# BaamPark/DistributedDataParallel-Cifar10

Measured on AMD Instinct MI355X. Metric: images/sec (whole node) CIFAR-10 ResNet at 1/2/4/8 MI355X; scaling efficiency, higher is better.
Workload: dtype bf16; 1 GPU; model=NetResDeep(n_chans1=32, n_blocks=10), global_batch=32, per_rank_batch=32, image=3x32x32, parallelism=dp1, optimizer=SGD(lr=1e-2)

## Files before the change

### distributeddataparallel_cifar10_amd/csrc/engine.hip

```cpp
#include <rccl/rccl.h>

#include <cstdio>
#include <cstdlib>
#include <cstring>
#include <map>
#include <string>
#include <vector>

#include "netresdeep_kernels.hip"
#include "xgmi_allreduce.hip"
#include "netresdeep_pks.hip"

namespace {

thread_local std::string g_err;

#define HIPCK(x)                                                                   \
  do {                                                                             \
    hipError_t e_ = (x);                                                           \
    if (e_ != hipSuccess) {                                                        \
      g_err = std::string(#x) + ": " + hipGetErrorString(e_);                      \
      return -1;                                                                   \
    }                                                                              \
  } while (0)
// ... 222 lines not shown
  else
    hipLaunchKernelGGL(xg::k_xgmi_ar_sgd<false>, dim3(xg::AR_NB), dim3(xg::AR_T), 0, e->st, cx, e->peers,
                       (const float*)cx.grads, (float*)nullptr, e->qa.err + 1, 1, e->ar_deadline);
  HIPCK(hipGetLastError());
  return 0;
}

static int pks_grid(int B) { return (B + 7) / 8 * 8 * pks::S; }
static int pks_live(int B) { return B * pks::S; }

static int coresident_budget(int per_cu, int ncu, int n_share, bool full_device) {
  const int slots = per_cu * ncu;
  const int margin = per_cu > 1 ? ncu : (full_device && n_share <= 1 ? 0 : 1);
  return (slots - margin) / std::max(n_share, 1);
}
static int share_budget(const Engine* e) {
  return e->shared_device > 1 ? coresident_budget(e->per_cu, e->ncu, e->shared_device, false) : e->resident;
}
static int seg_ch(const Engine* e) { return e->shared_device > 1 ? 256 : 128; }

static bool fc_in_step_for(const Engine* e, int B) {
  return e->fc_in_step && pks_live(B) + pks::N_FCW <= share_budget(e);
}
static int reduce_grid(const Engine* e, int nred_plus) {
  return e->shared_device > 1 ? std::min(nred_plus, share_budget(e)) : nred_plus;
}

static bool prologue_ok(const Engine* e, int B) {
  if (!e->persistent || !e->prologue) return false;
  if (e->comm_on && e->in.comm_mode != 2) return false;
  if (!fc_in_step_for(e, B)) return false;
  return pks_live(B) + std::max(pks::N_FCW, pks::prologue_segments(seg_ch(e))) <= share_budget(e);
}

static int enqueue_pks_step(Engine* e, int B, int s, bool prev) {
  Ctx cx = e->base;
  cx.B = B;
  const bool multi = e->comm_on, xgmi = multi && e->in.comm_mode == 2;
  if (xgmi && !e->peers_open) {
    g_err = "xGMI all-reduce: peers not mapped (call dca_engine_ipc_open first)";
    return -1;
  }
  if (pks_live(B) > share_budget(e)) {
    g_err = "persistent engine: " + std::to_string(pks_live(B)) + " step workgroups (batch " + std::to_string(B) +
            ") exceed the co-residency budget of " + std::to_string(share_budget(e)) + " per rank";
    return -1;
  }
  pks::RedAr ra{};
  ra.peers = e->peers;
  ra.err = e->qa.err + 1;
  ra.deadline = e->ar_deadline;
  ra.mode = !multi ? 0 : (xgmi ? 2 : 1);
  const bool fc = fc_in_step_for(e, B);
  ra.fc_in_step = pks::ra_flags(fc, prev, s, 0);
  ra.seg_ch = seg_ch(e);
  const int extra = fc ? std::max(pks::N_FCW, prev ? pks::prologue_segments(ra.seg_ch) : 0) : 0;
  const dim3 grid(pks_grid(B) + extra);
  const dim3 blk(pks::NTH);
  if (e->bf && prev)
    hipLaunchKernelGGL((pks::k_pks_step<0, true>), grid, blk, pks::Plan<0>::TOTAL, e->st, cx, e->qa, ra);
  else if (e->bf)
    hipLaunchKernelGGL((pks::k_pks_step<0, false>), grid, blk, pks::Plan<0>::TOTAL, e->st, cx, e->qa, ra);
  else if (prev)
    hipLaunchKernelGGL((pks::k_pks_step<1, true>), grid, blk, pks::Plan<1>::TOTAL, e->st, cx, e->qa, ra);
  else
    hipLaunchKernelGGL((pks::k_pks_step<1, false>), grid, blk, pks::Plan<1>::TOTAL, e->st, cx, e->qa, ra);
  HIPCK(hipGetLastError());
  return 0;
}

static int enqueue_pks_reduce(Engine* e, int B, int chunk, int part) {
  Ctx cx = e->base;
  cx.B = B;
  const bool multi = e->comm_on, xgmi = multi && e->in.comm_mode == 2;
  if (part != 2) {
    pks::RedAr ra{};
    ra.peers = e->peers;
    ra.err = e->qa.err + 1;
    ra.deadline = e->ar_deadline;
    ra.mode = !multi ? 0 : (xgmi ? 2 : 1);
    const bool fc = fc_in_step_for(e, B);
    ra.fc_in_step = pks::ra_flags(fc, false, 0, chunk);
    ra.seg_ch = seg_ch(e);
    const dim3 rgrid(reduce_grid(e, pks::reduce_segments(fc, ra.seg_ch) + 1));
    const int lean = !fc ? 0 : (ra.mode == 0 ? 1 : (ra.mode == 2 ? 2 : 0));
    const size_t lds = pks::stage_floats(B) * 4;
    if (lean == 1)
      hipLaunchKernelGGL(pks::k_pks_reduce_ar<1>, rgrid, dim3(256), lds, e->st, cx, e->qa, B * pks::S, ra);
    else if (lean == 2)
      hipLaunchKernelGGL(pks::k_pks_reduce_ar<2>, rgrid, dim3(256), lds, e->st, cx, e->qa, B * pks::S, ra);
    else
      hipLaunchKernelGGL(pks::k_pks_reduce_ar<0>, rgrid, dim3(256), lds, e->st, cx, e->qa, B * pks::S, ra);
  }
  if (multi && !xgmi) {
    if (part == 0) NCCK(ncclAllReduce(cx.grads, cx.grads, FLAT_N, ncclFloat32, ncclSum, e->comm, e->st));
    if (part != 1) hipLaunchKernelGGL(e->kapply, dim3(64), dim3(NT), 0, e->st, cx, 1);
  }
  HIPCK(hipGetLastError());
  return 0;
}

static int enqueue_step_persistent(Engine* e, int B, int part) {
  if (part != 2 && enqueue_pks_step(e, B, 0, false)) return -1;
  return enqueue_pks_reduce(e, B, 1, part);
}

static int enqueue_step(Engine* e, int B, int part = 0);
static int enqueue_chunk(Engine* e, int B, int chunk) {
  if (!prologue_ok(e, B)) {
    for (int s = 0; s < chunk; ++s)
      if (enqueue_step(e, B)) return -1;
    return 0;
  }
  for (int s = 0; s < chunk; ++s)
    if (enqueue_pks_step(e, B, s, s > 0)) return -1;
  return enqueue_pks_reduce(e, B, chunk, 0);
}

static int enqueue_step(Engine* e, int B, int part) {
  if (e->persistent) return enqueue_step_persistent(e, B, part);
  Ctx cx = e->base;
  cx.B = B;
  if (part == 2) {
    hipLaunchKernelGGL(e->kapply, dim3(64), dim3(NT), 0, e->st, cx, 1);
    HIPCK(hipGetLastError());
    return 0;
  }
  const int nparts = B * e->TPI, nw = B * (16 / e->RW);
  const int nslab = 9 * nw + nparts;
  const dim3 blk(NT);
  hipLaunchKernelGGL(e->kstem, dim3(nparts), blk, e->s_stem, e->st, cx);
  for (int i = 1; i < NBLK; ++i) hipLaunchKernelGGL(e->kfwd, dim3(nparts), blk, e->s_fwd, e->st, cx, i);
  hipLaunchKernelGGL(e->khead1, dim3(nparts), blk, e->s_head1, e->st, cx);
  hipLaunchKernelGGL(e->khead2, dim3(nparts), blk, e->s_head2, e->st, cx);
  for (int i = NBLK - 1; i >= 0; --i) {
    const int extra = (i == NBLK - 1) ? N_FC_WG : nw;
    size_t lds = (i == 0) ? e->s_dgrad0 : e->s_dgrad;
    lds = std::max(lds, (i < NBLK - 1) ? e->s_wgrad : e->s_fc);
    hipLaunchKernelGGL(e->kbwd, dim3(nparts + extra), blk, lds, e->st, cx, i);
    if (i == NBLK - 1 && e->comm_on && part == 0 && e->in.comm_mode == 0) {
      HIPCK(hipEventRecord(e->evA, e->st));
      HIPCK(hipStreamWaitEvent(e->cst, e->evA, 0));
      NCCK(ncclAllReduce(cx.grads, cx.grads, BUCKET_A_END, ncclFloat32, ncclSum, e->comm, e->cst));
    }
  }
  const int nother = cx.fuse_sgd ? 64 : 0;
  hipLaunchKernelGGL(e->kred, dim3(N_TRUNK_RED_WG + N_STEM_RED_WG + nother + 1), blk, 0, e->st, cx, nslab, nparts);
  if (e->comm_on && part == 0 && e->in.comm_mode == 2) return enqueue_xgmi_sgd(e, cx);
  if (e->comm_on && part == 0) {
    HIPCK(hipEventRecord(e->evB, e->st));
    HIPCK(hipStreamWaitEvent(e->cst, e->evB, 0));
    NCCK(ncclAllReduce(cx.grads + OFF_CONVW, cx.grads + OFF_CONVW, FLAT_N - OFF_CONVW, ncclFloat32, ncclSum, e->comm,
                       e->cst));
    HIPCK(hipEventRecord(e->evC, e->cst));
    HIPCK(hipStreamWaitEvent(e->st, e->evC, 0));
    hipLaunchKernelGGL(e->kapply, dim3(64), blk, 0, e->st, cx, 1);
  }
  HIPCK(hipGetLastError());
  return 0;
}

}


using dca::Engine;

extern "C" {

// ... 636 lines not shown
```

### distributeddataparallel_cifar10_amd/csrc/netresdeep_pks.hip

```cpp

namespace dca {
#ifndef DCA_DETAIL_FWD
#define DCA_DETAIL_FWD 5
#endif
#ifndef DCA_DETAIL_BWD
#define DCA_DETAIL_BWD 5
#endif
namespace pks {

constexpr int S = 4;
constexpr int RS = 16 / S;
constexpr int NW = 2 * RS;
constexpr int NTH = 64 * NW;
constexpr int GSTR = 64 + 2 * 512;
constexpr int LMAX = 64 * S;
constexpr int NNT = (18 + NW - 1) / NW;
constexpr int RND_HEAD = 10;
constexpr unsigned SPIN_LIMIT = 1u << 17;
constexpr int RB = 64;
constexpr int cmax(int a, int b) { return a > b ? a : b; }

struct Args {
  unsigned long long* gran;
  unsigned* bnx;
// ... 251 lines not shown
      if (ok) need &= ~(1u << k);
    }
#pragma unroll
    for (int p = 0; p < 2; ++p)
      if (xh[p][1] == htag && xh[p][3] == htag) need &= ~(1u << (8 + p));
    if (__all(need == 0)) break;
    if (spins >= SPIN_LIMIT) {
      if (lane == 0) atomicOr(pa.err, 1u << (round & 31));
      break;
    }
  }
#pragma unroll
  for (int e = 0; e < 4; ++e) sv[e] = 0.f;
#pragma unroll
  for (int k = 0; k < KS; ++k) {
    const bool valid = 4 * wv + sub + 4 * NW * k < G;
#pragma unroll
    for (int e = 0; e < 4; ++e) sv[e] += valid ? __uint_as_float(xa[k][e]) : 0.f;
  }
#pragma unroll
  for (int p = 0; p < 2; ++p) {
    hv[2 * p] = __uint_as_float(xh[p][0]);
    hv[2 * p + 1] = __uint_as_float(xh[p][2]);
  }
}
__device__ __forceinline__ void xchg_wait(const Args& pa, int round, int epoch, int G, float* cred, bool halo,
                                          int Lsrc, int which, int h, float (&hv)[4]) {
  const int t = threadIdx.x, lane = t & 63;
  const int wv = __builtin_amdgcn_readfirstlane(t >> 6);
  const unsigned tag = tagof(epoch, round);
  float sv[4];
  const unsigned btag = bn_tag(epoch, round);
  if (G <= 4 * NW) sweep_wait<1>(pa, round, wv, lane, G, btag, sv, halo, Lsrc, which, h, tag, hv);
  else if (G <= 8 * NW) sweep_wait<2>(pa, round, wv, lane, G, btag, sv, halo, Lsrc, which, h, tag, hv);
  else if (G <= 16 * NW) sweep_wait<4>(pa, round, wv, lane, G, btag, sv, halo, Lsrc, which, h, tag, hv);
  else sweep_wait<8>(pa, round, wv, lane, G, btag, sv, halo, Lsrc, which, h, tag, hv);
#pragma unroll
  for (int e = 0; e < 4; ++e) {
    sv[e] = xsum_rows(sv[e]);
  }
  if (lane < 16) {
#pragma unroll
    for (int e = 0; e < 4; ++e) cred[(4 * lane + e) * NW + wv] = sv[e];
  }
}
__device__ __forceinline__ float slot_total(const float* cred, int slot) {
  static_assert(NW == 8 && RS == 4, "slot-major combine layout: 8 waves, 4 rows");
  const f32x4 u = *(const f32x4*)(cred + slot * NW), w = *(const f32x4*)(cred + slot * NW + 4);
  float a = u[0];
  a += u[1];
  a += u[2];
  a += u[3];
  a += w[0];
  a += w[1];
  a += w[2];
  a += w[3];
  return a;
}

__device__ __forceinline__ void st4_wt(void* p, f32x4 v) {
  asm volatile("global_store_dwordx4 %0, %1, off sc1\n\ts_nop 1" ::"v"(p), "v"(v) : "memory");
}
__device__ __forceinline__ void st2_wt(float* p, float a, float b) {
  typedef float f2_ __attribute__((ext_vector_type(2)));
  asm volatile("global_store_dwordx2 %0, %1, off sc1" ::"v"(p), "v"(f2_{a, b}) : "memory");
}
__device__ __forceinline__ void st1_wt(float* p, float v) {
  __hip_atomic_store((unsigned*)p, __float_as_uint(v), __ATOMIC_RELAXED, __HIP_MEMORY_SCOPE_AGENT);
}
__device__ __forceinline__ void st4r_wt(float* rowp, int h, int lane, const float (&v)[4]) {
  st4_wt(rowp + h * 256 + lane * 4, f32x4{v[0], v[1], v[2], v[3]});
}
__device__ __forceinline__ void st4r(float* rowp, int h, int lane, const float (&v)[4]) {
  *(f32x4*)(rowp + h * 256 + lane * 4) = f32x4{v[0], v[1], v[2], v[3]};
}
__device__ __forceinline__ void ld4r(const float* rowp, int h, int lane, float (&v)[4]) {
  const f32x4 u = *(const f32x4*)(rowp + h * 256 + lane * 4);
  v[0] = u[0];
  v[1] = u[1];
  v[2] = u[2];
  v[3] = u[3];
}

template <int P>
__device__ __forceinline__ void wgrad_acc(const unsigned short* dyT, const unsigned short* xT, f32x4 (&wacc)[NNT][2],
                                          int wv, int lane) {
  using PL = Plan<P>;
  const int c = lane & 15, q = lane >> 4;
  constexpr int DYO = PL::DYT_PL / 2, XTO = PL::XT_PL / 2;
#pragma unroll
  for (int s = 0; s < RS / 2; ++s) {
    const int row = 2 * s + (q >> 1), c0 = 8 * (q & 1);
    const int ao0 = c * PL::DYT_S + row * 16 + c0, ao1 = (16 + c) * PL::DYT_S + row * 16 + c0;
    const bf16x8 a0 = *(const bf16x8*)(dyT + ao0);
    const bf16x8 a1 = *(const bf16x8*)(dyT + ao1);
    bf16x8 a0l = a0, a1l = a1;
    if constexpr (P == 1) {
      a0l = *(const bf16x8*)(dyT + DYO + ao0);
      a1l = *(const bf16x8*)(dyT + DYO + ao1);
    }
#pragma unroll
    for (int j = 0; j < NNT; ++j) {
      const int nt = wv + NW * j;
      if (nt < 18) {
        const int tap = nt >> 1, cih = nt & 1, kh = tap / 3, kw = tap % 3;
        const int bo = (kw * 32 + 16 * cih + c) * PL::XT_S + (row + kh) * 16 + c0;
        const bf16x8 b = *(const bf16x8*)(xT + bo);
        bf16x8 bl = b;
        if constexpr (P == 1) bl = *(const bf16x8*)(xT + XTO + bo);
        wacc[j][0] = mma3<P>(a0, a0l, b, bl, wacc[j][0]);
        wacc[j][1] = mma3<P>(a1, a1l, b, bl, wacc[j][1]);
      }
    }
  }
}
__device__ __forceinline__ void xt_put(unsigned short* xT, int XT_S, int xrow, int ch, int q, unsigned b0, unsigned b1,
                                       unsigned b2, unsigned b3) {
  const int rowoff = xrow * 16 + 4 * q;
  unsigned short* p1 = xT + (32 + ch) * XT_S + rowoff;
  *(uint2*)p1 = uint2{b0 | (b1 << 16), b2 | (b3 << 16)};
  unsigned short* p0 = xT + ch * XT_S + rowoff;
  p0[1] = (unsigned short)b0;
  *(unsigned*)(p0 + 2) = b1 | (b2 << 16);
  if (q < 3) p0[4] = (unsigned short)b3;
  unsigned short* p2 = xT + (64 + ch) * XT_S + rowoff;
  if (q > 0) p2[-1] = (unsigned short)b0;
  *(unsigned*)p2 = b1 | (b2 << 16);
  p2[2] = (unsigned short)b3;
}
template <int P>
__device__ __forceinline__ void xt_row(unsigned short* xT, int xrow, int q, int ch, const float (&x)[4]) {
  using PL = Plan<P>;
  unsigned hb[4], lb[4];
#pragma unroll
  for (int i = 0; i < 4; ++i) {
    const unsigned short hi = bfbits(x[i]);
    hb[i] = hi;
    lb[i] = P == 1 ? bf_lo(x[i], hi) : 0u;
  }
  xt_put(xT, PL::XT_S, xrow, ch, q, hb[0], hb[1], hb[2], hb[3]);
  if constexpr (P == 1) xt_put(xT + PL::XT_PL / 2, PL::XT_S, xrow, ch, q, lb[0], lb[1], lb[2], lb[3]);
}
template <int P>
__device__ __forceinline__ void xr_row(char* XR, int xrow, int q, int ch, const float (&v)[4]) {
  using PL = Plan<P>;
#pragma unroll
  for (int i = 0; i < 4; ++i) st1r<P>(XR, PL::XR_PL, xrow * 18 + 4 * q + i + 1, ch, v[i]);
}

template <int P>
__device__ __forceinline__ void wt_dma(char* wt, const unsigned short* src, int wv, int lane) {
  constexpr int BYTES = (P + 1) * PKW_PLANE * 2, NCH = (BYTES + 1023) / 1024;
  static_assert(BYTES == (P + 1) * Plan<P>::WT_PL, "record layout of pkw matches the LDS weight planes");
#pragma unroll
  for (int m = 0; m < (NCH + NW - 1) / NW; ++m) {
    const int ck = wv + NW * m;
    if (ck < NCH && ck * 1024 + lane * 16 < BYTES)
      __builtin_amdgcn_global_load_lds((const __attribute__((address_space(1))) void*)((const char*)src + ck * 1024 + lane * 16),
                                       (__attribute__((address_space(3))) void*)(wt + ck * 1024), 16, 0, 0);
  }
}
template <int P>
__device__ __forceinline__ void wt_copy_sc1(char* wt, const unsigned short* src) {
  constexpr int BYTES = (P + 1) * PKW_PLANE * 2, N16 = BYTES / 16, R = (N16 + NTH - 1) / NTH;
  const __amdgpu_buffer_rsrc_t rs = __builtin_amdgcn_make_buffer_rsrc((void*)src, (short)0, BYTES, 0x00020000);
  v4u v[R];
// ... 97 lines not shown
__host__ __device__ __forceinline__ int ra_chunk(const RedAr& ra) { return (ra.fc_in_step >> 16) & 255; }
__host__ __device__ __forceinline__ int ra_flags(int fc, int prev, int s, int chunk) {
  return (fc ? 1 : 0) | (prev ? 2 : 0) | (s << 8) | (chunk << 16);
}
__device__ __forceinline__ int step_epoch(const Args& pa, const RedAr& ra) {
  return (int)(((unsigned)*pa.epoch + (unsigned)ra_s(ra)) % EPOCH_WRAP);
}
__device__ __forceinline__ char* rbase(const RedAr& ra, int q) { return ra.peers.base[q] + xg::REGION_BYTES; }
__device__ __forceinline__ float* rslab(const RedAr& ra, int q, int par) {
  return (float*)(rbase(ra, q) + xg::FLAG_BYTES) + (size_t)par * xg::SLAB_FLOATS;
}

template <int NTH>
__device__ bool seg_exchange(const Ctx& cx, const RedAr& ra, int b, float* segv, int len, int off, int ep0, int* s_ep) {
  const int t = threadIdx.x, W = cx.ws, me = cx.rank;
  int* myflags = (int*)rbase(ra, me);
  const unsigned long long t_in = __builtin_amdgcn_s_memrealtime();
  if (t == 0) {
    s_ep[0] = xg::next_ep(ep0);
    s_ep[1] = xg::failed(ra.err);
  }
  __syncthreads();
  const int ep = s_ep[0], par = ep & 1;
  if (s_ep[1]) return false;
  constexpr int SYS = 17;
  const __amdgpu_buffer_rsrc_t mine =
      __builtin_amdgcn_make_buffer_rsrc(rslab(ra, me, par), (short)0, (int)(xg::SLAB_FLOATS * 4), 0x00020000);
  for (int k = 4 * t; k < len; k += 4 * NTH)
    __builtin_amdgcn_raw_buffer_store_b128(__builtin_bit_cast(xg::v4u, *(const f32x4*)(segv + k)), mine,
                                           4 * (off + k), 0, SYS);
  asm volatile("s_waitcnt vmcnt(0)" ::: "memory");
  __syncthreads();
  if (t < W) xg::flag_store((int*)rbase(ra, t) + me * NSEG_MAX + b, ep);
  if (t < W) xg::wait_flag(myflags + t * NSEG_MAX + b, ep, ra.deadline, ra.err);
  __syncthreads();
  if (t == 0) s_ep[1] = xg::failed(ra.err);
  __syncthreads();
  if (s_ep[1]) return false;
  if (t == 0 && b < seg_layout(ra.seg_ch).r_ts && ra.peers.ticks != nullptr) {
    atomicAdd(ra.peers.ticks, __builtin_amdgcn_s_memrealtime() - t_in);
    atomicAdd(ra.peers.ticks + 1, 1ull);
  }
  for (int k = 4 * t; k < len; k += 4 * NTH) {
    *(f32x4*)(segv + k) = rank_sum(W, [&](int q) {
      const __amdgpu_buffer_rsrc_t rs = __builtin_amdgcn_make_buffer_rsrc(rslab(ra, q, par), (short)0,
                                                                          (int)(xg::SLAB_FLOATS * 4), 0x00020000);
      return __builtin_bit_cast(f32x4, __builtin_amdgcn_raw_buffer_load_b128(rs, 4 * (off + k), 0, SYS));
    });
  }
  __syncthreads();
  return true;
}

__device__ __forceinline__ int seg_pidx(const SegLayout& G, int b, int k) {
  if (b < G.r_ts) {
    const bool stem = b >= G.r_trunk;
    const int e = (stem ? b - G.r_trunk : b) * G.ch + k, ii = k & 3;
    if (e >= (stem ? SSLAB_N : WSLAB_N)) return -1;
    const int tt = e >> 8, ln = (e >> 2) & 63, mt = tt & 1, nt = tt >> 1;
    if (!stem) return OFF_CONVW + (16 * mt + 4 * (ln >> 4) + ii) * 288 + (16 * (nt & 1) + (ln & 15)) * 9 + (nt >> 1);
    if (e < 1024) {
      const int kk = 16 * nt + (ln & 15);
      return kk < 27 ? OFF_C1W + (16 * mt + 4 * (ln >> 4) + ii) * 27 + kk : -1;
    }
    return e < 1056 ? OFF_C1B + (e - 1024) : -1;
  }
  if (b < G.fct) {
    const int fb = b - G.r_ts;
    return OFF_FC1W + (16 * (fb & 1) + (k >> 6)) * 2048 + 64 * (fb >> 1) + (k & 63);
  }
  if (b == G.fct) {
    if (k < 32) return OFF_FC1B + k;
    if (k < 352) return OFF_FC2W + ((k - 32) >> 5) * 32 + ((k - 32) & 31);
    return k < 362 ? OFF_FC2B + (k - 352) : -1;
  }
  return k < 64 ? (k < 32 ? OFF_BNW : OFF_BNB) + (k & 31) : -2 - (k - 64);
}

__device__ __forceinline__ f32x4 ld4_sc1(const float* base, int bytes, int off_floats) {
  const __amdgpu_buffer_rsrc_t rs = __builtin_amdgcn_make_buffer_rsrc((void*)base, (short)0, bytes, 0x00020000);
  return __builtin_bit_cast(f32x4, __builtin_amdgcn_raw_buffer_load_b128(rs, 4 * off_floats, 0, 16));
}

template <int NTH, int CH>
__device__ __forceinline__ void seg_chunk(const Ctx& cx, const Args& pa, const SegLayout& Ls, int b, int nslab,
                                          float* segv, f32x4* red) {
  constexpr int NS = CH / 4, VG = 2048 / CH, NG = NTH / NS, VPG = VG / NG, NU = 128 / VG, HG = VG / 2;
  static_assert(NG * VPG == VG && (VPG == 1 || VPG == 2), "512- or 256-thread reducers");
  const int t = threadIdx.x;
  const bool stem = b >= Ls.r_trunk;
  const int chunk = stem ? b - Ls.r_trunk : b;
  const int slot = t % NS, grp = t / NS, e0 = chunk * CH + slot * 4;
  const float* src = stem ? cx.SSLAB : pa.tslab;
  const int stride = stem ? SSLAB_N : WSLAB_N;
  const int ec = e0 < stride ? e0 : stride - 4;
  f32x4 sacc[VPG];
#pragma unroll
  for (int vp = 0; vp < VPG; ++vp) sacc[vp] = z4();
  for (int k0 = 0; k0 < nslab; k0 += 128) {
#pragma unroll
    for (int vp = 0; vp < VPG; ++vp) {
      const int gv = grp + NG * vp;
      f32x4 v[NU];
#pragma unroll
      for (int u = 0; u < NU; ++u) {
        const int k = k0 + gv + VG * u;
        const int kc = k < nslab ? k : nslab - 1;
        v[u] = ld4(src + (size_t)kc * stride + ec);
      }
#pragma unroll
      for (int u = 0; u < NU; ++u)
        if (k0 + gv + VG * u < nslab) sacc[vp] += v[u];
    }
  }
  red[t] = VPG == 2 ? sacc[0] + sacc[VPG - 1] : sacc[0];
  __syncthreads();
  if (t < NS) {
    f32x4 tot;
    if constexpr (VPG == 2) {
      tot = red[t];
#pragma unroll
      for (int g = 1; g < HG; ++g) tot += red[NS * g + t];
    } else {
      tot = red[t] + red[NS * HG + t];
#pragma unroll
      for (int g = 1; g < HG; ++g) tot += red[NS * g + t] + red[NS * (g + HG) + t];
    }
    *(f32x4*)(segv + slot * 4) = e0 < stride ? tot : z4();
  }
}

template <int NTH>
__device__ __forceinline__ void pkw_trunk_chunks_wt(const Ctx& cx, const float* wnew, int e_base, int len) {
  for (int t = threadIdx.x; t < 64 * (len / 128); t += NTH) {
    const int hf = t >> 6, j = t & 63, kind = j >> 4, idx = j & 15;
    const int e0 = e_base + hf * 128, tt = e0 >> 8, h = (e0 >> 7) & 1, mt = tt & 1, nt = tt >> 1;
    const int tap = nt >> 1, cih = nt & 1;
    const float* w = wnew + hf * 128;
    unsigned short v[8];
    int dst;
    if (kind < 2) {
      const int col = idx >> 1, qq = idx & 1, co = 16 * mt + 8 * h + col;
#pragma unroll
      for (int j8 = 0; j8 < 8; ++j8) {
        const float x = w[64 * (col >> 2) + 4 * (8 * qq + j8) + (col & 3)];
        const unsigned short hi = bfbits(x);
        v[j8] = kind == 0 ? hi : bf_lo(x, hi);
      }
      dst = (kind == 1 ? PKW_PLANE : 0) + pkw_elem(tap * 32 + co, 16 * cih + 8 * qq);
    } else {
      const int cl = idx;
#pragma unroll
      for (int c8 = 0; c8 < 8; ++c8) {
        const float x = w[64 * (c8 >> 2) + 4 * cl + (c8 & 3)];
        const unsigned short hi = bfbits(x);
        v[c8] = kind == 2 ? hi : bf_lo(x, hi);
      }
      dst = PKW_DGRAD + (kind == 3 ? PKW_PLANE : 0) + pkw_elem((8 - tap) * 32 + 16 * cih + cl, 16 * mt + 8 * h);
    }
    st4_wt(cx.pkw + dst, __builtin_bit_cast(f32x4, v4u{v[0] | ((unsigned)v[1] << 16), v[2] | ((unsigned)v[3] << 16),
                                                       v[4] | ((unsigned)v[5] << 16), v[6] | ((unsigned)v[7] << 16)}));
  }
}

template <int NTH, bool WT = false, int LEAN = 0>
__device__ void seg_process(const Ctx& cx, const Args& pa, const RedAr& ra, int b, int nslab, float* segv,
                            f32x4* red, float* stage, int* s_ep, int sslot, int swg) {
  const int t = threadIdx.x, B = cx.B;
  const int mode = LEAN == 1 ? 0 : (LEAN == 2 ? 2 : ra.mode);
  const SegLayout Ls = seg_layout(ra.seg_ch);
  const int len = seg_len(Ls, b), off = seg_off(Ls, b);
  const int ep0 = mode >= 2 && t == 0 ? xg::flag_load((const int*)rbase(ra, cx.rank) + cx.rank * NSEG_MAX + b) : 0;
  constexpr int KMAX = SEG_MAX / NTH;
  int pid[KMAX];
  float pold[KMAX];
#pragma unroll
  for (int i = 0; i < KMAX; ++i) {
    const int k = t + NTH * i;
    pid[i] = k < len && mode != 3 ? seg_pidx(Ls, b, k) : -1;
    pold[i] = cx.params[pid[i] >= 0 ? pid[i] : 0];
  }
  if (mode == 3) {
    for (int k = t; k < len; k += NTH) segv[k] = off + k < ra.st_n ? ra.st_src[off + k] : 0.f;
  } else if (b < Ls.r_ts) {
    if (Ls.ch == 128) seg_chunk<NTH, 128>(cx, pa, Ls, b, nslab, segv, red);
    else seg_chunk<NTH, 256>(cx, pa, Ls, b, nslab, segv, red);
  } else if (!LEAN && b < Ls.fct) {
    const int fb = b - Ls.r_ts, f = fb >> 1, j0 = 16 * (fb & 1);
    float* dh_s = stage;
    float* p_s = stage + B * 32;
    constexpr int MD = (64 * 8 + NTH - 1) / NTH, MP = (64 * 16 + NTH - 1) / NTH;
    f32x4 dh4[MD], p4[MP];
#pragma unroll
    for (int m = 0; m < MD; ++m) {
      const int idx = t + NTH * m;
      dh4[m] = ld4_sc1(cx.HDH, 64 * 32 * 4, 4 * (idx < B * 8 ? idx : 0));
    }
#pragma unroll
    for (int m = 0; m < MP; ++m) {
      const int idx = t + NTH * m, ic = idx < B * 16 ? idx : 0, bb = ic >> 4, k4 = ic & 15;
      p4[m] = ld4_sc1(cx.HP, 64 * 2048 * 4, bb * 2048 + 64 * f + 4 * k4);
    }
#pragma unroll
    for (int m = 0; m < MD; ++m)
      if (t + NTH * m < B * 8) st4(dh_s + 4 * (t + NTH * m), dh4[m]);
#pragma unroll
    for (int m = 0; m < MP; ++m)
      if (t + NTH * m < B * 16) st4(p_s + 4 * (t + NTH * m), p4[m]);
    __syncthreads();
    if (t < 256) {
      const int jl = t >> 4, kk = 4 * (t & 15);
      f32x4 a0 = z4();
#pragma unroll 8
      for (int bb = 0; bb < B; ++bb) a0 += dh_s[bb * 32 + j0 + jl] * ld4(p_s + bb * 64 + kk);
      st4(segv + jl * 64 + kk, a0);
    }
  } else if (!LEAN && b == Ls.fct) {
    float* hh_s = stage;
    float* dl_s = stage + B * 32;
    float* dh_s = dl_s + B * 16;
    for (int idx = t; idx < B * 8; idx += NTH) {
      st4(hh_s + 4 * idx, ld4_sc1(cx.HH, 64 * 32 * 4, 4 * idx));
      st4(dh_s + 4 * idx, ld4_sc1(cx.HDH, 64 * 32 * 4, 4 * idx));
    }
    for (int idx = t; idx < B * 10; idx += NTH) {
      const __amdgpu_buffer_rsrc_t rs = __builtin_amdgcn_make_buffer_rsrc((void*)cx.HDL, (short)0, 64 * 16 * 4, 0x00020000);
      dl_s[(idx / 10) * 16 + idx % 10] = __builtin_bit_cast(float, __builtin_amdgcn_raw_buffer_load_b32(rs, 4 * idx, 0, 16));
    }
    __syncthreads();
    for (int idx = t; idx < FCT_LEN; idx += NTH) {
      float sv = 0.f;
      if (idx < 32) {
#pragma unroll 8
        for (int bb = 0; bb < B; ++bb) sv += dh_s[bb * 32 + idx];
      } else if (idx < 352) {
        const int o = (idx - 32) >> 5, jj = (idx - 32) & 31;
#pragma unroll 8
        for (int bb = 0; bb < B; ++bb) sv += dl_s[bb * 16 + o] * hh_s[bb * 32 + jj];
      } else if (idx < 362) {
        const int o = idx - 352;
#pragma unroll 8
        for (int bb = 0; bb < B; ++bb) sv += dl_s[bb * 16 + o];
      }
      segv[idx] = sv;
    }
  } else {
    for (int idx = t; idx < BNT_LEN; idx += NTH) {
      float sv;
      if (idx < 64) {
        sv = pa.bng[idx];
      } else {
        const int k = idx - 64;
        sv = cx.rank == 0 ? (k < 32 ? cx.rm[k] : cx.rv[k - 32]) : 0.f;
      }
      segv[idx] = sv;
    }
  }
  __syncthreads();
  DCA_STAMP(cx, sslot, swg, 1);
  if (mode >= 2 && !seg_exchange<NTH>(cx, ra, b, segv, len, off, ep0, s_ep)) return;
  DCA_STAMP(cx, sslot, swg, 2);
#pragma unroll
  for (int i = 0; i < KMAX; ++i) {
    const int k = t + NTH * i;
    if (k >= len) break;
    const int pidx = pid[i];
    const float g = segv[k];
    if (mode == 3) {
      if (off + k < ra.st_n) ra.st_dst[off + k] = g;
// ... 596 lines not shown
    const f32x4 st4 = st4n;
    const float mean = st4[0], inv = st4[1], sc = st4[2], sh = st4[3];
#pragma unroll
    for (int i2 = 0; i2 < 4; ++i2) {
      const float z = __builtin_fmaf(yv[i2], sc, sh);
      x[i2] = x[i2] - fmaxf(z, 0.f);
      xh[i2] = (yv[i2] - mean) * inv;
      dz[i2] = z > 0.f ? g[i2] : 0.f;
      sa += dz[i2];
      sbv += dz[i2] * xh[i2];
      if (halo) {
        const float zo = __builtin_fmaf(yo[i2], sc, sh);
        xo[i2] = xo[i2] - fmaxf(zo, 0.f);
        xho[i2] = (yo[i2] - mean) * inv;
      }
    }
    const int rnd = RND_HEAD + 1 + (NBLK - 1 - i);
    const unsigned tag = tagof(epoch, rnd);
    if (i == DCA_DETAIL_BWD) DCA_STAMP(cx, 7, L, 0);
    const float pv = wg_csum(sa, sbv, cred);
    if (t < 64) bn_put(pa, rnd, L, t, bn_tag(epoch, rnd), pv);
    if (halo) publish_row(pa, rnd, L, hwhich, hh, tag, dz, lane);
    if (i == DCA_DETAIL_BWD) DCA_STAMP(cx, 7, L, 1);
    if (i < NBLK - 1) wgrad_acc<P>(dyT, xT, wacc, wv, lane);
    if (i == DCA_DETAIL_BWD) DCA_STAMP(cx, 7, L, 2);
    lds_barrier();
    xt_row<P>(xT, w + 1, q, ch, x);
    if (halo) xt_row<P>(xT, hxrow, q, ch, xo);
    float dzo[4];
    if (i == DCA_DETAIL_BWD) DCA_STAMP(cx, 7, L, 3);
    xchg_wait(pa, rnd, epoch, G, cred, halo, hsrc, hwhich ^ 1, hh, dzo);
    if (i == DCA_DETAIL_BWD) DCA_STAMP(cx, 7, L, 4);
    if (i > 0) {
      ld4r(cx.Y + (size_t)(i - 1) * B * 8192 + img8, hh, lane, yv);
    } else {
      codew = *(const unsigned*)(cx.SCODE + img8 + hh * 256 + lane * 4);
      {
        const int ci = t / 80, rem = t % 80, xr_ = rem >> 3, yimg = 8 * s - 1 + xr_;
        const int yc = yimg < 0 ? 0 : (yimg > 31 ? 31 : yimg);
        imgw = ((const unsigned*)my_img)[(ci < 3 ? ci : 2) * 256 + yc * 8 + (rem & 7)];
      }
      if (t < 48) nxt = ((const uint4*)(cx.data + (size_t)next_id * 3072 + 768 * s))[t];
      if (t == 48) nxt_lab = cx.labels[next_id];
    }
    if (halo && i > 0) ld4r(pa.yh + ((size_t)((i - 1) * LMAX + L) * 2 + hwhich) * 512, hh, lane, yo);
    lds_barrier();
    if (i == NBLK - 1 && ra_fc(ra) && t == 0) gput(pa.hdone + L, tagof(epoch, RND_HDONE), 0.f);
    if (i == DCA_DETAIL_BWD) DCA_STAMP(cx, 7, L, 5);
    if (L == 0 && t < 32) {
      dbet += slot_total(cred, t);
      dgam += slot_total(cred, 32 + t);
    }
    float dyv[4], dyo[4];
    {
      const float Sa = slot_total(cred, ch), Sb = slot_total(cred, 32 + ch);
      const float k1 = sc / Ntot;
#pragma unroll
      for (int i2 = 0; i2 < 4; ++i2) {
        dyv[i2] = k1 * (Ntot * dz[i2] - Sa - xh[i2] * Sb);
        if (halo) dyo[i2] = k1 * (Ntot * dzo[i2] - Sa - xho[i2] * Sb);
      }
    }
    xr_row<P>(XR, w + 1, q, ch, dyv);
    if (halo) xr_row<P>(XR, hxrow, q, ch, dyo);
    {
      unsigned hb[4], lb[4];
#pragma unroll
      for (int i2 = 0; i2 < 4; ++i2) {
        const unsigned short hi = bfbits(dyv[i2]);
        hb[i2] = hi;
        lb[i2] = P == 1 ? bf_lo(dyv[i2], hi) : 0u;
      }
      *(uint2*)(dyT + ch * PL::DYT_S + w * 16 + 4 * q) = uint2{hb[0] | (hb[1] << 16), hb[2] | (hb[3] << 16)};
      if constexpr (P == 1)
        *(uint2*)(dyT + PL::DYT_PL / 2 + ch * PL::DYT_S + w * 16 + 4 * q) =
            uint2{lb[0] | (lb[1] << 16), lb[2] | (lb[3] << 16)};
    }
    if (pa.debug) {
      st4r(cx.DY + (size_t)i * B * 8192 + img8, hh, lane, dyv);
      st4r(cx.X + (size_t)i * B * 8192 + img8, hh, lane, x);
    }
    lds_barrier();
    if (i == DCA_DETAIL_BWD) DCA_STAMP(cx, 7, L, 6);
    if (i > 0) st4n = stat[(i - 1) * 32 + ch];
    {
      const f32x4 acc = conv_row<P>(XR, WT, bw, w, hh, lane);
#pragma unroll
      for (int i2 = 0; i2 < 4; ++i2) g[i2] += acc[i2];
    }
    if (pa.debug && (i == 2 || i == 1)) st4r(cx.G + (size_t)(i == 2 ? 0 : 1) * B * 8192 + img8, hh, lane, g);
    DCA_STAMP(cx, 4 + (NBLK - 1 - i) / 8, L, (NBLK - 1 - i) % 8);
  }
  if (L == 0 && t < 32) {
    pa.bng[t] = dgam;
    pa.bng[32 + t] = dbet;
  }

  lds_barrier();
  wgrad_acc<P>(dyT, xT, wacc, wv, lane);
  DCA_STAMP(cx, 5, L, 2);
  {
    int tf = threadIdx.x;
    asm volatile("v_mov_b32 %0, %1" : "=v"(tf) : "v"(tf));
    const int t = tf, wv = tf >> 6, lane = tf & 63, c = lane & 15, q = lane >> 4;
    const int w = wv & (RS - 1), ch = 16 * (wv / RS) + c;
    unsigned short* dsT = (unsigned short*)(U + PL::U_DST);
    unsigned short* xs = (unsigned short*)(U + PL::U_XS);
    float* sred = (float*)(U + PL::U_SRED);
    float db = 0.f;
#pragma unroll
    for (int i2 = 0; i2 < 4; ++i2) {
      const unsigned code = (codew >> (8 * i2)) & 255u, pos = code & 3u;
      const float val = (code & 4u) ? g[i2] : 0.f;
      const unsigned short vh = bfbits(val);
      const unsigned vb = vh, vl = P == 1 ? (unsigned)bf_lo(val, vh) : 0u;
      const int so = ch * PL::DSP + (2 * w) * 32 + 2 * (4 * q + i2);
      *(unsigned*)(dsT + so) = (pos == 0 ? vb : 0u) | ((pos == 1 ? vb : 0u) << 16);
      *(unsigned*)(dsT + so + 32) = (pos == 2 ? vb : 0u) | ((pos == 3 ? vb : 0u) << 16);
      if constexpr (P == 1) {
        *(unsigned*)(dsT + PL::DST_PL / 2 + so) = (pos == 0 ? vl : 0u) | ((pos == 1 ? vl : 0u) << 16);
        *(unsigned*)(dsT + PL::DST_PL / 2 + so + 32) = (pos == 2 ? vl : 0u) | ((pos == 3 ? vl : 0u) << 16);
      }
      db += val;
    }
    if (t < 240) {
      const int ci = t / 80, rem = t % 80, xr_ = rem >> 3, x0 = 4 * (rem & 7), yimg = 8 * s - 1 + xr_;
      const bool valid = yimg >= 0 && yimg < 32;
      unsigned hb[4], lb[4];
#pragma unroll
      for (int b2 = 0; b2 < 4; ++b2) {
        const float v = valid ? norm_px((imgw >> (8 * b2)) & 255u, ci) : 0.f;
        const unsigned short hi = bfbits(v);
        hb[b2] = hi;
        lb[b2] = P == 1 ? bf_lo(v, hi) : 0u;
      }
#pragma unroll
      for (int p = 0; p <= P; ++p) {
        const unsigned* bb = p ? lb : hb;
        unsigned short* base = xs + p * (PL::XS_PL / 2);
        unsigned short* p1 = base + ((3 + ci) * PL::XSR + xr_) * PL::XS_S + x0;
        *(uint2*)p1 = uint2{bb[0] | (bb[1] << 16), bb[2] | (bb[3] << 16)};
        unsigned short* p0 = base + ((0 + ci) * PL::XSR + xr_) * PL::XS_S + x0;
        p0[1] = (unsigned short)bb[0];
        *(unsigned*)(p0 + 2) = bb[1] | (bb[2] << 16);
        if (x0 + 4 < 32) p0[4] = (unsigned short)bb[3];
        if (x0 == 0) p0[0] = 0;
        unsigned short* p2 = base + ((6 + ci) * PL::XSR + xr_) * PL::XS_S + x0;
        if (x0 > 0) p2[-1] = (unsigned short)bb[0];
        *(unsigned*)p2 = bb[1] | (bb[2] << 16);
        p2[2] = (unsigned short)bb[3];
        if (x0 == 28) p2[3] = 0;
      }
    }
    const float dbv = wg_csum<true>(db, 0.f, cred);
    DCA_STAMP(cx, 5, L, 3);
    float* ss = cx.SSLAB + (size_t)L * SSLAB_N;
    if (t < 32) ss[1024 + t] = dbv;
    {
      const int tile = wv & 3, mt = tile & 1, nt = tile >> 1, sr0 = 4 * (wv >> 2);
      const int kidx = 16 * nt + c, kk = kidx < 27 ? kidx : 0, ci = kk / 9, kh = (kk % 9) / 3, kw = kk % 3;
      const unsigned short* abase = dsT + (16 * mt + c) * PL::DSP + 8 * q;
      const unsigned short* bbase = xs + ((kw * 3 + ci) * PL::XSR + kh) * PL::XS_S + 8 * q;
      f32x4 acc2 = z4();
#pragma unroll
      for (int sr = sr0; sr < sr0 + 4; ++sr) {
        const bf16x8 a = *(const bf16x8*)(abase + sr * 32);
        const bf16x8 bb = *(const bf16x8*)(bbase + sr * PL::XS_S);
        bf16x8 al = a, bl = bb;
        if constexpr (P == 1) {
          al = *(const bf16x8*)(abase + PL::DST_PL / 2 + sr * 32);
          bl = *(const bf16x8*)(bbase + PL::XS_PL / 2 + sr * PL::XS_S);
        }
        acc2 = mma3<P>(a, al, bb, bl, acc2);
      }
      st4(sred + ((wv * 64 + lane) << 2), acc2);
    }
    lds_barrier();
    if (t < 256) {
      const int tile = t >> 6, ln = t & 63;
      st4_wt(ss + ((tile * 64 + ln) << 2), ld4(sred + ((tile * 64 + ln) << 2)) + ld4(sred + (((tile + 4) * 64 + ln) << 2)));
    }
  }
  DCA_STAMP(cx, 5, L, 4);
  if (t < 48) st4_wt((uint4*)(pa.simg + (size_t)((par ^ 1) * 64 + n) * 3072 + 768 * s) + t, __builtin_bit_cast(f32x4, nxt));
  if (t == 48 && s == 0) pa.slab[(par ^ 1) * 64 + n] = nxt_lab;
  int wvf = wv;
  asm volatile("v_mov_b32 %0, %1" : "=v"(wvf) : "v"(wvf));
#pragma unroll
  for (int j = 0; j < NNT; ++j) {
    const int nt = wvf + NW * j;
    if (nt < 18) {
      st4_wt(pa.tslab + (size_t)L * WSLAB_N + (((2 * nt) * 64 + lane) << 2), wacc[j][0]);
      st4_wt(pa.tslab + (size_t)L * WSLAB_N + (((2 * nt + 1) * 64 + lane) << 2), wacc[j][1]);
    }
  }
  DCA_STAMP(cx, 5, L, 7);
}

template <int P, bool PRO>
__global__ void __launch_bounds__(NTH) k_pks_step(Ctx cx, Args pa, RedAr ra) {
  extern __shared__ __attribute__((aligned(16))) char smem[];
  const int gmain = (cx.B + 7) / 8 * 8 * S;
  if ((int)blockIdx.x < gmain) {
    step_main<P, PRO>(cx, pa, ra, smem);
    return;
  }
  const int fb = (int)blockIdx.x - gmain;
  if constexpr (PRO) {
    if (ra_prev(ra)) {
      prologue_reduce<P>(cx, pa, ra, fb, smem);
      __syncthreads();
    }
  }
  if (!ra_fc(ra)) return;
  const int nfw = min((int)gridDim.x - gmain, N_FCW);
  for (int f = fb; f < N_FCW; f += nfw) {
    if (f != fb) __syncthreads();
    fc_segment<P>(cx, pa, ra, f, smem);
  }
}


__global__ void __launch_bounds__(256) k_pks_prime(Ctx cx, Args pa) {
  const int t = threadIdx.x, b = blockIdx.x, par = *pa.epoch & 1, id = sample_id(cx, b);
  if (t < 192)
    ((uint4*)(pa.simg + (size_t)(par * 64 + b) * 3072))[t] = ((const uint4*)(cx.data + (size_t)id * 3072))[t];
  if (t == 192) pa.slab[par * 64 + b] = cx.labels[id];
}

__host__ __device__ inline int reduce_segments(int fc_in_step, int seg_ch) {
  return fc_in_step ? seg_layout(seg_ch).r_ts + 1 : seg_layout(seg_ch).nseg;
}

template <int LEAN>
__global__ void __launch_bounds__(256) k_pks_reduce_ar(Ctx cx, Args pa, int nslab, RedAr ra) {
  __shared__ __attribute__((aligned(16))) float segv[SEG_MAX];
  __shared__ f32x4 red[256];
  extern __shared__ __attribute__((aligned(16))) float stage[];
  __shared__ int s_ep[2];
  const int nred = reduce_segments(ra_fc(ra), ra.seg_ch), b = blockIdx.x, nwg = gridDim.x;
  const SegLayout Ls = seg_layout(ra.seg_ch);
  if (nwg > nred) {
    if (b >= nred) {
      if (ra.mode != 3) pks_bookkeeping(cx, pa, ra_chunk(ra));
      return;
    }
    const int seg = !ra_fc(ra) || b < Ls.r_ts ? b : Ls.bnt;
    DCA_STAMP(cx, 8, b, 0);
    seg_process<256, false, LEAN>(cx, pa, ra, seg, nslab, segv, red, stage, s_ep, 8, b);
    return;
  }
  for (int k = b; k < nred; k += nwg) {
    const int seg = !ra_fc(ra) || k < Ls.r_ts ? k : Ls.bnt;
    seg_process<256, false, LEAN>(cx, pa, ra, seg, nslab, segv, red, stage, s_ep, 8, k);
    __syncthreads();
  }
  if (b == nwg - 1 && ra.mode != 3) pks_bookkeeping(cx, pa, ra_chunk(ra));
}

}
}
```

Measured before the change: 394,800 images/sec.

## Split single-GPU reduce segments in half and interleave stem slab stores

In the single-rank lean reduce path, each trunk weight-gradient segment is now split into two halves processed by separate workgroups, doubling the reduce grid so more CUs share the slab summation. Separately, the stem backward now issues its weight-slab stores in three batches spread across its compute stages instead of all at the end, so the global writes overlap with later work. The split relies on the offset and length logic for halves matching the parameter index mapping, and it adds more workgroup launch and parameter-gather overhead for each half.

```diff
diff --git a/distributeddataparallel_cifar10_amd/csrc/engine.hip b/distributeddataparallel_cifar10_amd/csrc/engine.hip
--- a/distributeddataparallel_cifar10_amd/csrc/engine.hip
+++ b/distributeddataparallel_cifar10_amd/csrc/engine.hip
@@ -328,8 +328,8 @@
     const bool fc = fc_in_step_for(e, B);
     ra.fc_in_step = pks::ra_flags(fc, false, 0, chunk);
     ra.seg_ch = seg_ch(e);
-    const dim3 rgrid(reduce_grid(e, pks::reduce_segments(fc, ra.seg_ch) + 1));
     const int lean = !fc ? 0 : (ra.mode == 0 ? 1 : (ra.mode == 2 ? 2 : 0));
+    const dim3 rgrid(reduce_grid(e, pks::reduce_segments(fc, ra.seg_ch, lean) + 1));
     const size_t lds = pks::stage_floats(B) * 4;
     if (lean == 1)
       hipLaunchKernelGGL(pks::k_pks_reduce_ar<1>, rgrid, dim3(256), lds, e->st, cx, e->qa, B * pks::S, ra);
diff --git a/distributeddataparallel_cifar10_amd/csrc/netresdeep_pks.hip b/distributeddataparallel_cifar10_amd/csrc/netresdeep_pks.hip
--- a/distributeddataparallel_cifar10_amd/csrc/netresdeep_pks.hip
+++ b/distributeddataparallel_cifar10_amd/csrc/netresdeep_pks.hip
@@ -620,15 +620,15 @@
   return __builtin_bit_cast(f32x4, __builtin_amdgcn_raw_buffer_load_b128(rs, 4 * off_floats, 0, 16));
 }
 
-template <int NTH, int CH>
+template <int NTH, int CH, int PARTS = 1>
 __device__ __forceinline__ void seg_chunk(const Ctx& cx, const Args& pa, const SegLayout& Ls, int b, int nslab,
-                                          float* segv, f32x4* red) {
-  constexpr int NS = CH / 4, VG = 2048 / CH, NG = NTH / NS, VPG = VG / NG, NU = 128 / VG, HG = VG / 2;
+                                          float* segv, f32x4* red, int part = 0) {
+  constexpr int NS = CH / 4 / PARTS, VG = 2048 / CH, NG = NTH / NS, VPG = VG / NG, NU = 128 / VG, HG = VG / 2;
   static_assert(NG * VPG == VG && (VPG == 1 || VPG == 2), "512- or 256-thread reducers");
   const int t = threadIdx.x;
   const bool stem = b >= Ls.r_trunk;
   const int chunk = stem ? b - Ls.r_trunk : b;
-  const int slot = t % NS, grp = t / NS, e0 = chunk * CH + slot * 4;
+  const int slot = t % NS, grp = t / NS, e0 = chunk * CH + (part * NS + slot) * 4;
   const float* src = stem ? cx.SSLAB : pa.tslab;
   const int stride = stem ? SSLAB_N : WSLAB_N;
   const int ec = e0 < stride ? e0 : stride - 4;
@@ -703,11 +703,12 @@
 
 template <int NTH, bool WT = false, int LEAN = 0>
 __device__ void seg_process(const Ctx& cx, const Args& pa, const RedAr& ra, int b, int nslab, float* segv,
-                            f32x4* red, float* stage, int* s_ep, int sslot, int swg) {
+                            f32x4* red, float* stage, int* s_ep, int sslot, int swg, int half = -1) {
   const int t = threadIdx.x, B = cx.B;
   const int mode = LEAN == 1 ? 0 : (LEAN == 2 ? 2 : ra.mode);
   const SegLayout Ls = seg_layout(ra.seg_ch);
-  const int len = seg_len(Ls, b), off = seg_off(Ls, b);
+  const int len = LEAN == 1 && half >= 0 ? Ls.ch / 2 : seg_len(Ls, b), off = seg_off(Ls, b);
+  const int koff = LEAN == 1 && half > 0 ? len : 0;
   const int ep0 = mode >= 2 && t == 0 ? xg::flag_load((const int*)rbase(ra, cx.rank) + cx.rank * NSEG_MAX + b) : 0;
   constexpr int KMAX = SEG_MAX / NTH;
   int pid[KMAX];
@@ -715,14 +716,19 @@
 #pragma unroll
   for (int i = 0; i < KMAX; ++i) {
     const int k = t + NTH * i;
-    pid[i] = k < len && mode != 3 ? seg_pidx(Ls, b, k) : -1;
+    pid[i] = k < len && mode != 3 ? seg_pidx(Ls, b, koff + k) : -1;
     pold[i] = cx.params[pid[i] >= 0 ? pid[i] : 0];
   }
   if (mode == 3) {
     for (int k = t; k < len; k += NTH) segv[k] = off + k < ra.st_n ? ra.st_src[off + k] : 0.f;
   } else if (b < Ls.r_ts) {
-    if (Ls.ch == 128) seg_chunk<NTH, 128>(cx, pa, Ls, b, nslab, segv, red);
-    else seg_chunk<NTH, 256>(cx, pa, Ls, b, nslab, segv, red);
+    if constexpr (LEAN == 1) {
+      if (Ls.ch == 128) seg_chunk<NTH, 128, 2>(cx, pa, Ls, b, nslab, segv, red, half);
+      else seg_chunk<NTH, 256, 2>(cx, pa, Ls, b, nslab, segv, red, half);
+    } else {
+      if (Ls.ch == 128) seg_chunk<NTH, 128>(cx, pa, Ls, b, nslab, segv, red);
+      else seg_chunk<NTH, 256>(cx, pa, Ls, b, nslab, segv, red);
+    }
   } else if (!LEAN && b < Ls.fct) {
     const int fb = b - Ls.r_ts, f = fb >> 1, j0 = 16 * (fb & 1);
     float* dh_s = stage;
@@ -1507,6 +1513,20 @@
     asm volatile("v_mov_b32 %0, %1" : "=v"(tf) : "v"(tf));
     const int t = tf, wv = tf >> 6, lane = tf & 63, c = lane & 15, q = lane >> 4;
     const int w = wv & (RS - 1), ch = 16 * (wv / RS) + c;
+    asm volatile("s_waitcnt vmcnt(0)" ::: "memory");
+    pin(codew);
+    pin(imgw);
+    pin(nxt);
+    pin(nxt_lab);
+    auto slab_store = [&](int j) {
+      const int nt = wv + NW * j;
+      if (nt < 18) {
+        st4_wt(pa.tslab + (size_t)L * WSLAB_N + (((2 * nt) * 64 + lane) << 2), wacc[j][0]);
+        st4_wt(pa.tslab + (size_t)L * WSLAB_N + (((2 * nt + 1) * 64 + lane) << 2), wacc[j][1]);
+      }
+    };
+    static_assert(NNT == 3, "three pairs of slab stores, one per stage of the stem backward");
+    slab_store(0);
     unsigned short* dsT = (unsigned short*)(U + PL::U_DST);
     unsigned short* xs = (unsigned short*)(U + PL::U_XS);
     float* sred = (float*)(U + PL::U_SRED);
@@ -1555,6 +1575,7 @@
         if (x0 == 28) p2[3] = 0;
       }
     }
+    slab_store(1);
     const float dbv = wg_csum<true>(db, 0.f, cred);
     DCA_STAMP(cx, 5, L, 3);
     float* ss = cx.SSLAB + (size_t)L * SSLAB_N;
@@ -1578,6 +1599,7 @@
       }
       st4(sred + ((wv * 64 + lane) << 2), acc2);
     }
+    slab_store(2);
     lds_barrier();
     if (t < 256) {
       const int tile = t >> 6, ln = t & 63;
@@ -1587,16 +1609,6 @@
   DCA_STAMP(cx, 5, L, 4);
   if (t < 48) st4_wt((uint4*)(pa.simg + (size_t)((par ^ 1) * 64 + n) * 3072 + 768 * s) + t, __builtin_bit_cast(f32x4, nxt));
   if (t == 48 && s == 0) pa.slab[(par ^ 1) * 64 + n] = nxt_lab;
-  int wvf = wv;
-  asm volatile("v_mov_b32 %0, %1" : "=v"(wvf) : "v"(wvf));
-#pragma unroll
-  for (int j = 0; j < NNT; ++j) {
-    const int nt = wvf + NW * j;
-    if (nt < 18) {
-      st4_wt(pa.tslab + (size_t)L * WSLAB_N + (((2 * nt) * 64 + lane) << 2), wacc[j][0]);
-      st4_wt(pa.tslab + (size_t)L * WSLAB_N + (((2 * nt + 1) * 64 + lane) << 2), wacc[j][1]);
-    }
-  }
   DCA_STAMP(cx, 5, L, 7);
 }
 
@@ -1631,8 +1643,9 @@
   if (t == 192) pa.slab[par * 64 + b] = cx.labels[id];
 }
 
-__host__ __device__ inline int reduce_segments(int fc_in_step, int seg_ch) {
-  return fc_in_step ? seg_layout(seg_ch).r_ts + 1 : seg_layout(seg_ch).nseg;
+__host__ __device__ inline int reduce_segments(int fc_in_step, int seg_ch, int lean = 0) {
+  return lean == 1 ? 2 * seg_layout(seg_ch).r_ts + 1
+                   : (fc_in_step ? seg_layout(seg_ch).r_ts + 1 : seg_layout(seg_ch).nseg);
 }
 
 template <int LEAN>
@@ -1641,21 +1654,24 @@
   __shared__ f32x4 red[256];
   extern __shared__ __attribute__((aligned(16))) float stage[];
   __shared__ int s_ep[2];
-  const int nred = reduce_segments(ra_fc(ra), ra.seg_ch), b = blockIdx.x, nwg = gridDim.x;
+  const int nred = reduce_segments(ra_fc(ra), ra.seg_ch, LEAN), b = blockIdx.x, nwg = gridDim.x;
   const SegLayout Ls = seg_layout(ra.seg_ch);
+  auto seg_of = [&](int k) {
+    if constexpr (LEAN == 1) return k < 2 * Ls.r_ts ? k >> 1 : Ls.bnt;
+    return !ra_fc(ra) || k < Ls.r_ts ? k : Ls.bnt;
+  };
+  auto half_of = [&](int k) { return LEAN == 1 && k < 2 * Ls.r_ts ? k & 1 : -1; };
   if (nwg > nred) {
     if (b >= nred) {
       if (ra.mode != 3) pks_bookkeeping(cx, pa, ra_chunk(ra));
       return;
     }
-    const int seg = !ra_fc(ra) || b < Ls.r_ts ? b : Ls.bnt;
     DCA_STAMP(cx, 8, b, 0);
-    seg_process<256, false, LEAN>(cx, pa, ra, seg, nslab, segv, red, stage, s_ep, 8, b);
+    seg_process<256, false, LEAN>(cx, pa, ra, seg_of(b), nslab, segv, red, stage, s_ep, 8, b, half_of(b));
     return;
   }
   for (int k = b; k < nred; k += nwg) {
-    const int seg = !ra_fc(ra) || k < Ls.r_ts ? k : Ls.bnt;
-    seg_process<256, false, LEAN>(cx, pa, ra, seg, nslab, segv, red, stage, s_ep, 8, k);
+    seg_process<256, false, LEAN>(cx, pa, ra, seg_of(k), nslab, segv, red, stage, s_ep, 8, k, half_of(k));
     __syncthreads();
   }
   if (b == nwg - 1 && ra.mode != 3) pks_bookkeeping(cx, pa, ra_chunk(ra));
```

New measurement: 398,700 images/sec (median of 6 runs). About the same (+1.0%).

## Move wgrad accumulation into last backward iteration and interleave slab stores

Applied to the files above, without the earlier changes.

The weight-gradient accumulation now runs inside the final backward-loop iteration (i==0) instead of after the loop. Its six per-wave slab tile stores are spread across the later stem-gradient work rather than issued in one burst at the end. The intent is to overlap global write-through stores with LDS/MMA work and shorten the kernel tail. The segment reducer also issues all slab loads for both groups before accumulating, to raise memory-level parallelism. Register pressure rises from holding more loads and wacc live across the stem section, and the ordering relies on wgrad_acc seeing final dyT/xT at i==0.

```diff
diff --git a/distributeddataparallel_cifar10_amd/csrc/netresdeep_pks.hip b/distributeddataparallel_cifar10_amd/csrc/netresdeep_pks.hip
--- a/distributeddataparallel_cifar10_amd/csrc/netresdeep_pks.hip
+++ b/distributeddataparallel_cifar10_amd/csrc/netresdeep_pks.hip
@@ -357,6 +357,13 @@
   v[3] = u[3];
 }
 
+__device__ __forceinline__ void slab_store(const Args& pa, int L, int j, int mt, const f32x4& v) {
+  int tf = threadIdx.x;
+  asm volatile("v_mov_b32 %0, %1" : "=v"(tf) : "v"(tf));
+  const int nt = ((tf >> 6) & (NW - 1)) + NW * j;
+  if (nt < 18) st4_wt(pa.tslab + (size_t)L * WSLAB_N + (((2 * nt + mt) * 64 + (tf & 63)) << 2), v);
+}
+
 template <int P>
 __device__ __forceinline__ void wgrad_acc(const unsigned short* dyT, const unsigned short* xT, f32x4 (&wacc)[NNT][2],
                                           int wv, int lane) {
@@ -636,19 +643,23 @@
 #pragma unroll
   for (int vp = 0; vp < VPG; ++vp) sacc[vp] = z4();
   for (int k0 = 0; k0 < nslab; k0 += 128) {
+    f32x4 v[VPG][NU];
 #pragma unroll
     for (int vp = 0; vp < VPG; ++vp) {
       const int gv = grp + NG * vp;
-      f32x4 v[NU];
 #pragma unroll
       for (int u = 0; u < NU; ++u) {
         const int k = k0 + gv + VG * u;
         const int kc = k < nslab ? k : nslab - 1;
-        v[u] = ld4(src + (size_t)kc * stride + ec);
-      }
+        v[vp][u] = ld4(src + (size_t)kc * stride + ec);
+      }
+    }
+#pragma unroll
+    for (int vp = 0; vp < VPG; ++vp) {
+      const int gv = grp + NG * vp;
 #pragma unroll
       for (int u = 0; u < NU; ++u)
-        if (k0 + gv + VG * u < nslab) sacc[vp] += v[u];
+        if (k0 + gv + VG * u < nslab) sacc[vp] += v[vp][u];
     }
   }
   red[t] = VPG == 2 ? sacc[0] + sacc[VPG - 1] : sacc[0];
@@ -1485,6 +1496,17 @@
     }
     lds_barrier();
     if (i == DCA_DETAIL_BWD) DCA_STAMP(cx, 7, L, 6);
+    if (i == 0) {
+      wgrad_acc<P>(dyT, xT, wacc, wv, lane);
+      DCA_STAMP(cx, 5, L, 5);
+      pin(codew);
+      pin(imgw);
+      pin(nxt);
+      pin(nxt_lab);
+      static_assert(NNT == 3, "six slab tiles per wave, stored one by one");
+      slab_store(pa, L, 0, 0, wacc[0][0]);
+      DCA_STAMP(cx, 5, L, 6);
+    }
     if (i > 0) st4n = stat[(i - 1) * 32 + ch];
     {
       const f32x4 acc = conv_row<P>(XR, WT, bw, w, hh, lane);
@@ -1499,8 +1521,8 @@
     pa.bng[32 + t] = dbet;
   }
 
+  slab_store(pa, L, 0, 1, wacc[0][1]);
   lds_barrier();
-  wgrad_acc<P>(dyT, xT, wacc, wv, lane);
   DCA_STAMP(cx, 5, L, 2);
   {
     int tf = threadIdx.x;
@@ -1526,6 +1548,7 @@
       }
       db += val;
     }
+    slab_store(pa, L, 1, 0, wacc[1][0]);
     if (t < 240) {
       const int ci = t / 80, rem = t % 80, xr_ = rem >> 3, x0 = 4 * (rem & 7), yimg = 8 * s - 1 + xr_;
       const bool valid = yimg >= 0 && yimg < 32;
@@ -1555,10 +1578,12 @@
         if (x0 == 28) p2[3] = 0;
       }
     }
+    slab_store(pa, L, 1, 1, wacc[1][1]);
     const float dbv = wg_csum<true>(db, 0.f, cred);
     DCA_STAMP(cx, 5, L, 3);
     float* ss = cx.SSLAB + (size_t)L * SSLAB_N;
     if (t < 32) ss[1024 + t] = dbv;
+    slab_store(pa, L, 2, 0, wacc[2][0]);
     {
       const int tile = wv & 3, mt = tile & 1, nt = tile >> 1, sr0 = 4 * (wv >> 2);
       const int kidx = 16 * nt + c, kk = kidx < 27 ? kidx : 0, ci = kk / 9, kh = (kk % 9) / 3, kw = kk % 3;
@@ -1578,6 +1603,7 @@
       }
       st4(sred + ((wv * 64 + lane) << 2), acc2);
     }
+    slab_store(pa, L, 2, 1, wacc[2][1]);
     lds_barrier();
     if (t < 256) {
       const int tile = t >> 6, ln = t & 63;
@@ -1587,16 +1613,6 @@
   DCA_STAMP(cx, 5, L, 4);
   if (t < 48) st4_wt((uint4*)(pa.simg + (size_t)((par ^ 1) * 64 + n) * 3072 + 768 * s) + t, __builtin_bit_cast(f32x4, nxt));
   if (t == 48 && s == 0) pa.slab[(par ^ 1) * 64 + n] = nxt_lab;
-  int wvf = wv;
-  asm volatile("v_mov_b32 %0, %1" : "=v"(wvf) : "v"(wvf));
-#pragma unroll
-  for (int j = 0; j < NNT; ++j) {
-    const int nt = wvf + NW * j;
-    if (nt < 18) {
-      st4_wt(pa.tslab + (size_t)L * WSLAB_N + (((2 * nt) * 64 + lane) << 2), wacc[j][0]);
-      st4_wt(pa.tslab + (size_t)L * WSLAB_N + (((2 * nt + 1) * 64 + lane) << 2), wacc[j][1]);
-    }
-  }
   DCA_STAMP(cx, 5, L, 7);
 }
 
```

Result: no change. 394,800 images/sec before, 397,900 images/sec after (median of 6 runs) (+0.8%).
